# evandez/neuron-descriptions

Hardware: AMD Instinct MI355X
Metric: neuron-descriptions/sec (whole node), 4096 neurons x k=15 exemplars (higher is better)
Workload: dtype f32-equivalent: operands split into (hi,lo) f16 pairs (22 significant bits), 3 f16 MFMAs per product, f32 accumulate

## Files before the change

include/milan_hip.h:

```cpp
#ifndef MILAN_HIP_H
#define MILAN_HIP_H

#include <stddef.h>
#include <stdint.h>

#ifdef __cplusplus
extern "C" {
#endif

#if defined(__GNUC__)
#pragma GCC visibility push(default)
#endif

#define MILAN_ABI_VERSION 11

enum {
  MILAN_OK = 0,
  MILAN_ERR_ARG = -1,
  MILAN_ERR_SHAPE = -2,
  MILAN_ERR_STATE = -3,
  MILAN_ERR_WORKSPACE = -4,
  MILAN_ERR_NO_LM = -5
};

// ... 190 lines not shown
typedef struct milan_sketch_op {
  int32_t kind, src, dst, offset, extremes, reserved;
  int64_t n, position, capacity;
} milan_sketch_op;
int milan_exemplar_sketch_plan_shift(int64_t resolution, int64_t buffersize,
                                     int full_rate, int n_levels,
                                     const int64_t* capacities,
                                     const int64_t* firstfree,
                                     int (*draw_bit)(void*), void* user,
                                     milan_sketch_op* ops, int max_ops, int* n_ops,
                                     int64_t* capacities_out, int64_t* firstfree_out,
                                     int* n_levels_out);

int milan_exemplar_sketch_quantile(const float* const* levels,
                                   const int64_t* firstfree,
                                   const int64_t* capacities, int n_levels,
                                   int n_units, float* extremes, float q,
                                   float* out, void* workspace,
                                   size_t workspace_bytes, milan_stream stream);

int milan_exemplar_render(const float* hiddens, int batch, int channels, int h,
                          int w, const float* images, int img_h, int img_w,
                          const int32_t* cells, int n_cells, const float* levels,
                          const float* mul3, const float* add3, int out_size,
                          int k, uint8_t* out_images, uint8_t* out_masks,
                          uint8_t* out_masked, milan_stream stream);

int milan_conv2d_nhwc(const float* x, int n, int h, int w, int cin,
                      const float* weight_oihw, const float* bias, int cout,
                      int kh, int kw, int stride, int pad, int relu,
                      const float* residual, float* y, int precision,
                      milan_stream stream);

size_t milan_lm_train_workspace_bytes(const milan_ctx* ctx, int rows, int L);
int milan_lm_nll(milan_ctx* ctx, const float* const* params, int n_params,
                 const int64_t* inputs, const int64_t* targets, int rows, int L,
                 float* loss_sum_and_count, void* workspace,
                 size_t workspace_bytes, milan_stream stream);
int milan_lm_train_step(milan_ctx* ctx, const float* const* params,
                        float* const* grads, int n_params,
                        const int64_t* inputs, const int64_t* targets, int rows,
                        int L, float dropout, uint64_t seed,
                        float* loss_sum_and_count, void* workspace,
                        size_t workspace_bytes, milan_stream stream);

size_t milan_decoder_train_workspace_bytes(const milan_ctx* ctx, int rows,
                                           int k, int L);
int milan_decoder_nll(milan_ctx* ctx, const float* const* params, int n_params,
                      const float* features, const int64_t* targets, int rows,
                      int k, int L, float* loss_terms, void* workspace,
                      size_t workspace_bytes, milan_stream stream);
int milan_decoder_train_step(milan_ctx* ctx, const float* const* params,
                             float* const* grads, int n_params,
                             const float* features, const int64_t* targets,
                             int rows, int k, int L, float dropout,
                             uint64_t seed, float regularization_weight,
                             float* loss_terms, void* workspace,
                             size_t workspace_bytes, milan_stream stream);

size_t milan_decoder_grad_workspace_bytes(const milan_ctx* ctx, int rows, int k,
                                          int L);
int milan_decoder_forward_train(milan_ctx* ctx, const float* const* params,
                                int n_params, const float* features,
                                const int64_t* targets, int rows, int k, int L,
                                float dropout, uint64_t seed,
                                float* logprobs_out, float* attentions_out,
// ... 63 lines not shown
```

neuron-descriptions_amd/csrc/api.hip:

```cpp
#include "common.h"

#include <cstdarg>
#include <cstdio>
#include <cstring>

namespace milan {

static thread_local char g_err[1024] = "";

void set_error(const char* fmt, ...) {
  va_list ap;
  va_start(ap, fmt);
  vsnprintf(g_err, sizeof(g_err), fmt, ap);
  va_end(ap);
}

int dev_alloc(milan_ctx* c, void** p, size_t bytes) {
  if (bytes == 0) bytes = 16;
  MILAN_CHECK_HIP(hipMalloc(p, (bytes + 255) & ~size_t(255)));
  c->owned.push_back(*p);
  return 0;
}

__global__ void absmax_kernel(const float* __restrict__ w, long n,
// ... 333 lines not shown
    for (auto& g : c->graphs)
      if (g.exec) (void)hipGraphExecDestroy(g.exec);
    c->graphs.clear();
  }
  return 0;
}

int milan_graph_stats(const milan_ctx* c, long long* captures, long long* replays) {
  MILAN_REQUIRE(c, MILAN_ERR_ARG, "null ctx");
  if (captures) *captures = c->graph_captures;
  if (replays) *replays = c->graph_replays;
  return 0;
}

int milan_lm_score(milan_ctx* c, const int64_t* seqs, int rows, int L,
                   const int32_t* seq_len, float* out, void* workspace,
                   size_t workspace_bytes, milan_stream stream) {
  MILAN_REQUIRE(c && seqs && out, MILAN_ERR_ARG, "milan_lm_score: null argument");
  set_status_word(c->status);
  Arena a;
  MILAN_TRY(make_arena(workspace, workspace_bytes, &a));
  return decoder_lm_score(c, seqs, rows, L, seq_len, out, a, (hipStream_t)stream);
}

int milan_lm_logprobs(milan_ctx* c, const int64_t* seqs, int rows, int L,
                      float* out, void* workspace, size_t workspace_bytes,
                      milan_stream stream) {
  MILAN_REQUIRE(c && seqs && out, MILAN_ERR_ARG,
                "milan_lm_logprobs: null argument");
  set_status_word(c->status);
  Arena a;
  MILAN_TRY(make_arena(workspace, workspace_bytes, &a));
  return decoder_lm_logprobs(c, seqs, rows, L, out, a, (hipStream_t)stream);
}

int milan_conv2d_nhwc(const float* x, int n, int h, int w, int cin,
                      const float* weight_oihw, const float* bias, int cout,
                      int kh, int kw, int stride, int pad, int relu,
                      const float* residual, float* y, int precision,
                      milan_stream stream) {
  MILAN_REQUIRE(x && weight_oihw && y, MILAN_ERR_ARG, "conv2d: null argument");
  set_status_word(nullptr);
  const bool force_strip = precision == 3, tap_major = precision == 4;
  if (force_strip || tap_major) precision = MILAN_PRECISION_SPLIT_F16;
  MILAN_REQUIRE(!force_strip || MILAN_EXPERIMENTS, MILAN_ERR_ARG,
                "conv2d: the LDS-strip 3x3 kernel is only in an experiments build "
                "(make EXPERIMENTS=1)");
  MILAN_REQUIRE(precision == MILAN_PRECISION_F32 || cin % 32 == 0,
                MILAN_ERR_SHAPE, "conv2d: split-f16 needs cin %% 32 == 0");
  MILAN_REQUIRE(cin % 4 == 0 && n > 0 && cout > 0, MILAN_ERR_SHAPE,
                "conv2d: cin must be a multiple of 4");
  hipStream_t s = (hipStream_t)stream;
  const int K = kh * kw * cin, Kp = (K + 31) / 32 * 32;
  float *wp = nullptr, *zero = nullptr, *xs = nullptr, *wsp = nullptr, *ws3 = nullptr, *wst = nullptr;
  MILAN_CHECK_HIP(hipMalloc((void**)&wp, sizeof(float) * (size_t)cout * Kp));
  MILAN_CHECK_HIP(hipMalloc((void**)&zero, 256));
  MILAN_CHECK_HIP(hipMemsetAsync(zero, 0, 256, s));
  int r = pack_conv_plain(weight_oihw, cout, cin, kh, kw, wp, s);
  if (r == 0) {
    GemmArgs g{};
    const int ho = (h + 2 * pad - kh) / stride + 1, wo = (w + 2 * pad - kw) / stride + 1;
    g.A = x; g.W = wp; g.bias = bias; g.aux = residual; g.C = y;
    g.M = n * ho * wo; g.N = cout; g.K = K; g.Kp = Kp; g.ldc = cout; g.ldaux = cout;
    g.H = h; g.Wd = w; g.Cin = cin; g.Ho = ho; g.Wo = wo; g.KH = kh; g.KW = kw;
    g.stride = stride; g.pad = pad; g.a_pix_stride = cin;
    g.a_img_stride = (long)h * w * cin;
// ... 175 lines not shown
```

neuron-descriptions_amd/csrc/common.h:

```cpp
#pragma once
#include <hip/hip_runtime.h>
#include <stdint.h>
#include <stddef.h>
#include <string>
#include <vector>
#include <map>

#include "../../include/milan_hip.h"

#ifndef MILAN_EXPERIMENTS
#define MILAN_EXPERIMENTS 0
#endif

namespace milan {

void set_error(const char* fmt, ...);
#define MILAN_CHECK_HIP(expr)                                              \
  do {                                                                     \
    hipError_t _e = (expr);                                                \
    if (_e != hipSuccess) {                                                \
      milan::set_error("%s:%d: %s -> %s", __FILE__, __LINE__, #expr,       \
                       hipGetErrorString(_e));                             \
      return (int)_e;                                                      \
    }                                                                      \
// ... 373 lines not shown
int dev_alloc(milan_ctx* c, void** p, size_t bytes);
int make_split_weight(milan_ctx* c, const float* w, int n, int kp, float** ws,
                      float* ws_inv, hipStream_t s);
int pack_conv_plain(const float* w_oihw, int cout, int cin, int kh, int kw,
                    float* wp, hipStream_t s);
int encoder_finalize(milan_ctx* c, hipStream_t s);
int encoder_rescale(milan_ctx* c, hipStream_t s);
int make_slice_major(const float* ws, int cout, int taps, int cin, int gps, int gb, float* dst,
                     hipStream_t s);
int make_chunk_major(const float* ws, int cout, int cin, float* dst,
                     hipStream_t s);
size_t encoder_workspace(const milan_ctx* c, int n_images, int H, int W);
int encoder_run_spatial(milan_ctx* c, const void* images, int image_dtype,
                        const void* masks, int mask_dtype, int n, int H, int W,
                        float* out, milan::Arena& ws, hipStream_t s);
int encoder_run(milan_ctx* c, const void* images, int image_dtype,
                const void* masks, int mask_dtype, int n_images, int H, int W,
                float* features, Arena& ws, hipStream_t s);
int decoder_finalize(milan_ctx* c, hipStream_t s);
size_t decoder_workspace(const milan_ctx* c, int n, int k, int beam, int length);
int decoder_init_state(milan_ctx* c, const float* features, int n, int k,
                       float* h, float* cc, Arena& ws, hipStream_t s);
int decoder_step(milan_ctx* c, const float* features, int rows, int k,
                 const int64_t* tokens, const float* h, const float* cc,
                 float* h_lm, float* c_lm, float temperature,
                 float* predictions, float* attentions, float* h_out,
                 float* c_out, Arena& ws, hipStream_t s);
int decoder_decode(milan_ctx* c, const float* features, int n, int k,
                   int strategy, int length, int beam, int mi,
                   float temperature, int group_size, int64_t* tokens,
                   float* scores, float* predictions, float* attentions,
                   int64_t* beam_tokens, float* beam_scores, int32_t* out_len,
                   Arena& ws, hipStream_t s);
int decoder_lm_logprobs(milan_ctx* c, const int64_t* seqs, int rows, int L,
                        float* out, milan::Arena& ws, hipStream_t s);
int decoder_lm_score(milan_ctx* c, const int64_t* seqs, int rows, int L,
                     const int32_t* seq_len, float* out, Arena& ws,
                     hipStream_t s);
}
```

neuron-descriptions_amd/csrc/decoder.hip:

```cpp
#include "common.h"
#include <limits>
#include <optional>

namespace milan {

static constexpr float kFloatMin = -3.402823466e+38f;

static const Tensor* find(milan_ctx* c, const std::string& name) {
  auto it = c->raw.find(name);
  return it == c->raw.end() ? nullptr : &it->second;
}

__global__ void pack_rows_kernel(const float* __restrict__ src, int n, int k,
                                 int kp, float* __restrict__ dst) {
  const long total = (long)n * kp;
  for (long idx = blockIdx.x * (long)blockDim.x + threadIdx.x; idx < total;
       idx += (long)gridDim.x * blockDim.x) {
    const int r = idx / kp, col = idx - (long)r * kp;
    dst[idx] = col < k ? src[(long)r * k + col] : 0.f;
  }
}

__device__ inline int lstm_source_row(int i, int hidden) {
  if (!hidden) return i;
  const int gate = (i & 63) >> 4, u = (i >> 6) * 16 + (i & 15);
  return gate * hidden + u;
}
__global__ void add_vec_kernel(const float* a, const float* b, int n,
                               float* out, int hidden = 0) {
  const int i = blockIdx.x * blockDim.x + threadIdx.x;
  if (i < n) {
    const int r = lstm_source_row(i, hidden);
    out[i] = a[r] + (b ? b[r] : 0.f);
// ... 567 lines not shown
    sy = block_sum(sy, red);
    const float lsy = logf(sy);
    for (int i = tid; i < V; i += 256)
      pred[i] = ((pred[i] - mx) - ls) - lambda * ((y[i] - my) - lsy);
  } else {
    for (int i = tid; i < V; i += 256) pred[i] = (pred[i] - mx) - ls;
  }
  if (pred_out) {
    float* po = pred_out + (long)r * pred_stride;
    for (int i = tid; i < V; i += 256) po[i] = pred[i];
  }
  if (k <= 0) return;
  __syncthreads();
  if (last_tok && last_tok[r] == stop) {
    for (int j = tid; j < k; j += 256) {
      cand_v[(long)r * k + j] = j == 0 ? 0.f : kFloatMin;
      cand_i[(long)r * k + j] = j == 0 ? stop : (j - 1 < stop ? j - 1 : j);
    }
    return;
  }
  if (k >= 2 && k <= 256)
    block_topk_fast(pred, V, k, cand_v + (long)r * k, cand_i + (long)r * k,
                    reinterpret_cast<unsigned*>(sm + V + 8));
  else
    block_topk(pred, V, k, cand_v + (long)r * k, cand_i + (long)r * k, red, redi);
}

constexpr int kRowRegs = 24;

__device__ inline float funkey(unsigned key) {
  return __uint_as_float((key & 0x80000000u) ? (key ^ 0x80000000u) : ~key);
}

__global__ __launch_bounds__(256) void row_select_reg_kernel(
    const float* __restrict__ logits, const float* __restrict__ lm_logits,
    float lambda, int V, int k, const int64_t* __restrict__ last_tok, int stop,
    float* __restrict__ cand_v, int* __restrict__ cand_i,
    float* __restrict__ pred_out, long pred_stride, int rank_select) {
  __shared__ float red[8];
  __shared__ unsigned scratch[528];
  const int r = blockIdx.x, tid = threadIdx.x;
  const float* x = logits + (long)r * V;
  float p[kRowRegs];
  float mx = -INFINITY;
#pragma unroll
  for (int j = 0; j < kRowRegs; ++j) {
    const int i = tid + 256 * j;
    p[j] = i < V ? x[i] : -INFINITY;
    mx = fmaxf(mx, p[j]);
  }
  mx = block_max(mx, red);
  float s = 0.f;
#pragma unroll
  for (int j = 0; j < kRowRegs; ++j)
    if (tid + 256 * j < V) s += expf(p[j] - mx);
  s = block_sum(s, red);
  const float ls = logf(s);
  if (lm_logits) {
    const float* y = lm_logits + (long)r * V;
    float q[kRowRegs];
    float my = -INFINITY;
#pragma unroll
    for (int j = 0; j < kRowRegs; ++j) {
      const int i = tid + 256 * j;
      q[j] = i < V ? y[i] : -INFINITY;
      my = fmaxf(my, q[j]);
    }
// ... 5 lines not shown
    sy = block_sum(sy, red);
    const float lsy = logf(sy);
#pragma unroll
    for (int j = 0; j < kRowRegs; ++j)
      p[j] = ((p[j] - mx) - ls) - lambda * ((q[j] - my) - lsy);
  } else {
#pragma unroll
    for (int j = 0; j < kRowRegs; ++j) p[j] = (p[j] - mx) - ls;
  }
  if (pred_out) {
    float* po = pred_out + (long)r * pred_stride;
#pragma unroll
    for (int j = 0; j < kRowRegs; ++j)
      if (tid + 256 * j < V) po[tid + 256 * j] = p[j];
  }
  if (k <= 0) return;
  float* out_v = cand_v + (long)r * k;
  int* out_i = cand_i + (long)r * k;
  if (last_tok && last_tok[r] == stop) {
    for (int j = tid; j < k; j += 256) {
      out_v[j] = j == 0 ? 0.f : kFloatMin;
      out_i[j] = j == 0 ? stop : (j - 1 < stop ? j - 1 : j);
    }
    return;
  }
  unsigned key[kRowRegs];
#pragma unroll
  for (int j = 0; j < kRowRegs; ++j)
    key[j] = tid + 256 * j < V ? fkey(p[j]) : 0u;
  unsigned* cnt = scratch;
  float* cv = reinterpret_cast<float*>(scratch + 8);
  int* ci = reinterpret_cast<int*>(scratch + 8 + 256);
  if (k >= 2) {
    __shared__ unsigned gk[kGatherCap];
    __shared__ float gp[kGatherCap];
    __shared__ int gi[kGatherCap];
    __shared__ unsigned wave_t[4], gcount;
    unsigned tmax = 0u;
#pragma unroll
    for (int j = 0; j < kRowRegs; ++j) tmax = max(tmax, key[j]);
    const int m_need = (k + 3) >> 2;
    const int lane = tid & 63;
    int rank = 0;
#pragma unroll
    for (int u = 0; u < 64; ++u) {
      const unsigned m = (unsigned)__builtin_amdgcn_readlane((int)tmax, u);
      rank += (m > tmax) || (m == tmax && u < lane);
    }
    if (tid == 0) gcount = 0u;
    if (rank == m_need - 1) wave_t[tid >> 6] = rank_select ? tmax : 0u;
    __syncthreads();
    const unsigned T0 = min(min(wave_t[0], wave_t[1]), min(wave_t[2], wave_t[3]));
    if (T0 != 0u) {
#pragma unroll
      for (int j = 0; j < kRowRegs; ++j)
        if (key[j] >= T0) {
          const unsigned q = atomicAdd(&gcount, 1u);
          if (q < (unsigned)kGatherCap) { gk[q] = key[j]; gp[q] = p[j]; gi[q] = tid + 256 * j; }
        }
      __syncthreads();
      const int total = (int)gcount;
      if (total <= kGatherCap) {
        for (int c0 = tid; c0 < total; c0 += 256) {
          const unsigned mk = gk[c0];
          const int mi = gi[c0];
          int r2 = 0;
          for (int u = 0; u < total; ++u) {
            const unsigned ok = gk[u];
            r2 += (ok > mk) || (ok == mk && gi[u] < mi);
          }
          if (r2 < k) { out_v[r2] = gp[c0]; out_i[r2] = mi; }
        }
        return;
      }
    }
    __syncthreads();
  }
  unsigned kmax = 0u, kmin = 0xFFFFFFFFu;
#pragma unroll
  for (int j = 0; j < kRowRegs; ++j)
    if (tid + 256 * j < V) { kmax = max(kmax, key[j]); kmin = min(kmin, key[j]); }
  for (int o = 32; o > 0; o >>= 1) {
    kmax = max(kmax, (unsigned)__shfl_xor((int)kmax, o));
    kmin = min(kmin, (unsigned)__shfl_xor((int)kmin, o));
  }
  __syncthreads();
  if ((tid & 63) == 0) { cnt[tid >> 6] = kmax; cnt[4 + (tid >> 6)] = kmin; }
  __syncthreads();
  unsigned hi = max(max(cnt[0], cnt[1]), max(cnt[2], cnt[3]));
  unsigned lo = min(min(cnt[4], cnt[5]), min(cnt[6], cnt[7]));
  if (k == 1) {
    int best = 0x7fffffff;
#pragma unroll
    for (int j = 0; j < kRowRegs; ++j)
      if (key[j] == hi && tid + 256 * j < V) best = min(best, tid + 256 * j);
    for (int o = 32; o > 0; o >>= 1) best = min(best, __shfl_xor(best, o));
    __syncthreads();
    if ((tid & 63) == 0) cnt[tid >> 6] = (unsigned)best;
    __syncthreads();
    if (tid == 0) {
      out_i[0] = (int)min(min(cnt[0], cnt[1]), min(cnt[2], cnt[3]));
      out_v[0] = funkey(hi);
    }
    return;
  }
  for (int it = 0; it < 32 && lo < hi; ++it) {
// ... 563 lines not shown
                                      w.n, w.k, EPI_BIAS, c->zero);
      if (cell) { g.C2 = cn; g.Cs = hs2; }
      g.a_split = 1;
      g.acc_scale = w.ws_inv;
      g.Cin = ldx;
      g.A2 = hs; g.K1 = ldx; g.H2 = 1; g.W2d = 1; g.stride2 = 1;
      g.a2_pix_stride = H; g.a2_img_stride = H;
      MILAN_TRY(launch_gemm(g, s));
      if (!cell) {
        hipLaunchKernelGGL(lstm_pointwise_kernel, dim3(nblk((long)rows * H)),
                           dim3(256), 0, s, b->gates, cc, rows, H, hn, cn);
        hs2 = hs;
        MILAN_TRY(launch_f32_to_split(hn, H, hs2, H, rows, H, 1.f, s));
      }
    }
    hs = hs2;
    MILAN_TRY(launch_gemm(split_lin(c->out, b->logits, V, EPI_BIAS, nullptr, 0), s));
    MILAN_CHECK_HIP(hipGetLastError());
    return 0;
  }
  MILAN_TRY(lin(c, h, H, c->q2h, b->q, A, rows, EPI_BIAS, s));
  launch_attend(b->q, keys, c->att_w, c->att_b, rows, rpn, k, A, b->att, s);
  launch_context(b->att, features, rows, rpn, k, F, b->ctx, s);
  MILAN_TRY(lin(c, h, H, c->gate, b->x + E, ldx, rows, EPI_BIAS_SIGMUL, s, b->ctx, F));
  hipLaunchKernelGGL(embed_kernel, dim3(nblk((long)rows * E)), dim3(256), 0, s,
                     c->embedding, tok, rows, E, b->x, ldx);
  MILAN_TRY(lstm_layer(c, b->x, ldx, c->lstm_ih, h, H, c->lstm_hh, c->lstm_cat,
                       b->gates, cc, hn, cn, rows, s));
  MILAN_TRY(lin(c, hn, H, c->out, b->logits, V, rows, EPI_BIAS, s));
  MILAN_CHECK_HIP(hipGetLastError());
  return 0;
}

static size_t row_select_lds(int V) { return sizeof(float) * (V + 8 + 528); }

static int launch_row_select(const float* logits, const float* lm_logits,
                             float lambda, int rows, int V, int k,
                             const int64_t* last_tok, int stop, float* cand_v,
                             int* cand_i, float* pred_out, long pred_stride,
                             hipStream_t s) {
  if (V <= kRowRegs * 256 && k <= 256 && (k <= 1 || k <= V)) {
    static const int rank_select = [] {
      const char* e = getenv("MILAN_ROW_SELECT");
      return (e && e[0] == 't') ? 0 : 1;
    }();
    hipLaunchKernelGGL(row_select_reg_kernel, dim3(rows), dim3(256), 0, s,
                       logits, lm_logits, lambda, V, k, last_tok, stop, cand_v,
                       cand_i, pred_out, pred_stride, rank_select);
    MILAN_CHECK_HIP(hipGetLastError());
    return 0;
  }
  const size_t lds = row_select_lds(V);
  MILAN_REQUIRE(lds <= 160 * 1024, MILAN_ERR_SHAPE,
                "vocab_size %d too large for the row-select kernel", V);
  if (lds > 64 * 1024)
    MILAN_TRY(ensure_lds_attr(reinterpret_cast<const void*>(row_select_kernel), (int)lds));
  hipLaunchKernelGGL(row_select_kernel, dim3(rows), dim3(256), lds, s, logits,
                     lm_logits, lambda, V, k, last_tok, stop, cand_v, cand_i,
                     pred_out, pred_stride);
  MILAN_CHECK_HIP(hipGetLastError());
  return 0;
}

int decoder_step(milan_ctx* c, const float* features, int rows, int k,
                 const int64_t* tokens, const float* h, const float* cc,
                 float* h_lm, float* c_lm, float temperature, float* predictions,
                 float* attentions, float* h_out, float* c_out, Arena& ws,
                 hipStream_t s) {
  MILAN_TRY(check_dims(c, k));
  const bool mi = h_lm != nullptr;
  MILAN_REQUIRE((h_lm == nullptr) == (c_lm == nullptr), MILAN_ERR_ARG,
                "state must have both h_lm and c_lm or neither");
  MILAN_REQUIRE(!mi || c->d.has_lm, MILAN_ERR_NO_LM,
                "state has h_lm or c_lm, but decoder has no lm");
  DecBuf b;
  dec_plan(c, rows, k, 1, 1, mi, ws, &b);
  c->scratch = ws.off <= ws.size ? b.scratch : nullptr;
  c->scratch_floats = b.scratch_floats;
  MILAN_REQUIRE(ws.off <= ws.size, MILAN_ERR_WORKSPACE,
                "step: workspace too small (%zu needed)", ws.off);
  MILAN_TRY(project_keys(c, features, rows * k, b.keys, s));
  MILAN_TRY(step_core(c, features, b.keys, rows, 1, k, tokens, h, cc, h_out,
                      c_out, &b, s));
  const float* lm_logits = nullptr;
  if (mi) {
    LmState st{h_lm, c_lm, rows};
    MILAN_TRY(lm_step(c, tokens, rows, st, b.lm[0], b.lm_emb, b.lm_gates,
                      b.lm_logits, s));
    const size_t bytes = sizeof(float) * (size_t)rows * c->d.lm_hidden_size *
                         c->d.lm_layers;
    MILAN_CHECK_HIP(hipMemcpyAsync(h_lm, b.lm[0].h, bytes, hipMemcpyDeviceToDevice, s));
    MILAN_CHECK_HIP(hipMemcpyAsync(c_lm, b.lm[0].c, bytes, hipMemcpyDeviceToDevice, s));
    lm_logits = b.lm_logits;
  }
// ... 183 lines not shown
  const size_t state = (2 * (size_t)d.lm_layers + 1) * R * d.lm_hidden_size;
  return maps + state + 4 * R + 2048;
}

static int lm_score_dedup(milan_ctx* c, const int64_t* seqs, int rows, int L, int group,
                          const int32_t* seq_len, int len_div, float* total, DecBuf* b,
                          float* scratch, hipStream_t s) {
  const milan_dims& d = c->d;
  const int Hl = d.lm_hidden_size, El = d.lm_embedding_size, V = d.vocab_size;
  const int R = rows, G = (rows + group - 1) / group, nb = (V + 63) / 64;
  char* base = reinterpret_cast<char*>(scratch);
  size_t off = 0;
  auto take = [&](size_t bytes) { void* q = base + off; off += (bytes + 255) & ~size_t(255); return q; };
  int* rep = (int*)take(sizeof(int) * (size_t)(L + 1) * R);
  int* lrank = (int*)take(sizeof(int) * (size_t)(L + 1) * R);
  int* cnt = (int*)take(sizeof(int) * (size_t)(L + 1) * G);
  int* offs = (int*)take(sizeof(int) * (size_t)(L + 1) * G);
  LmDedup q;
  q.cls = (int*)take(sizeof(int) * (size_t)(L + 1) * R);
  q.urow = (int*)take(sizeof(int) * (size_t)(L + 1) * R);
  q.par = (int*)take(sizeof(int) * (size_t)(L + 1) * R);
  q.U = (int*)take(sizeof(int) * (size_t)(L + 1));
  q.gh = (float*)take(sizeof(float) * (size_t)d.lm_layers * R * Hl);
  q.gc = (float*)take(sizeof(float) * (size_t)d.lm_layers * R * Hl);
  q.gv = (float*)take(sizeof(float) * (size_t)R * Hl);
  q.tok_c = (int64_t*)take(sizeof(int64_t) * (size_t)R);
  q.tgt_c = (int64_t*)take(sizeof(int64_t) * (size_t)R);
  hipLaunchKernelGGL(lm_prefix_classes_kernel, dim3(G), dim3(256), 0, s, seqs, L, group, R, G,
                     rep, lrank, cnt);
  hipLaunchKernelGGL(lm_prefix_scan_kernel, dim3(L + 1), dim3(256), 0, s, cnt, G, offs, q.U);
  hipLaunchKernelGGL(lm_prefix_assign_kernel, dim3(nblk(R)), dim3(256), 0, s, rep, lrank, offs,
                     L, group, R, G, q.cls, q.urow, q.par);
  MILAN_CHECK_HIP(hipGetLastError());
  const size_t st_floats = (size_t)d.lm_layers * R * Hl;
  MILAN_TRY(launch_zero_fill(q.gh, sizeof(float) * st_floats, s));
  MILAN_TRY(launch_zero_fill(q.gc, sizeof(float) * st_floats, s));
  float* hs = b->lm_gates;
  float* emb_s = c->scratch;
  const size_t layer_sz = (size_t)R * Hl;
  int cur = 0;
  for (int t = 0; t + 1 < L; ++t) {
    const int p1 = t + 1, p2 = t + 2;
    const int* U1 = q.U + p1;
    const int* U2 = q.U + p2;
    LmState& st = b->lm[cur];
    LmState& nx = b->lm[cur ^ 1];
    hipLaunchKernelGGL(lm_gather_tok_kernel, dim3(nblk(R)), dim3(256), 0, s, seqs, (long)L, t,
                       q.urow + (size_t)p1 * R, U1, q.tok_c);
    hipLaunchKernelGGL(embed_split_kernel, dim3(nblk((long)R * (El / 8))), dim3(256), 0, s,
                       c->lm_embedding, q.tok_c, R, El, emb_s, El, U1);
    if (t > 0) {
      for (int l = 0; l < d.lm_layers; ++l) {
        hipLaunchKernelGGL(lm_gather_rows_kernel, dim3(nblk((long)R * (Hl / 4), 8192)), dim3(256),
                           0, s, (const float4*)(hs + ((size_t)cur * d.lm_layers + l) * layer_sz),
                           q.par + (size_t)p1 * R, U1, Hl / 4, (float4*)(q.gh + l * layer_sz));
        hipLaunchKernelGGL(lm_gather_rows_kernel, dim3(nblk((long)R * (Hl / 4), 8192)), dim3(256),
                           0, s, (const float4*)(st.c + (long)l * st.rows * Hl),
                           q.par + (size_t)p1 * R, U1, Hl / 4, (float4*)(q.gc + l * layer_sz));
      }
    }
    const float* in = emb_s;
    int in_dim = El;
    for (int l = 0; l < d.lm_layers; ++l) {
      float* h_next = hs + ((size_t)(cur ^ 1) * d.lm_layers + l) * layer_sz;
      float* hn = nx.h + (long)l * nx.rows * Hl;
      float* cn = nx.c + (long)l * nx.rows * Hl;
      const LinearW& w = c->lm_cat[l];
      GemmArgs g = linear_args(in, in_dim, w.ws, w.b, hn, Hl, R, w.n, w.k, EPI_LSTM, c->zero,
                               q.gc + l * layer_sz, Hl);
      g.C2 = cn; g.Cs = h_next;
      g.a_split = 1;
      g.acc_scale = w.ws_inv;
// ... 9 lines not shown
                       (const float4*)in, q.par + (size_t)p2 * R, U2, Hl / 4, (float4*)q.gv);
    hipLaunchKernelGGL(lm_gather_tok_kernel, dim3(nblk(R)), dim3(256), 0, s, seqs, (long)L, t + 1,
                       q.urow + (size_t)p2 * R, U2, q.tgt_c);
    {
      GemmArgs g = linear_args(q.gv, Hl, c->lm_out.ws, c->lm_out.b, b->lm_logits, V, R,
                               c->lm_out.n, c->lm_out.k, EPI_BIAS, c->zero);
      g.a_split = 1;
      g.acc_scale = c->lm_out.ws_inv;
      g.epilogue = EPI_LSE;
      g.ldc = 2 * nb;
      g.lse_tgt = reinterpret_cast<const long long*>(q.tgt_c);
      g.lse_tgt_stride = 1;
      g.lse_x = b->lm_logits + (size_t)R * 2 * nb;
      g.m_live = U2; g.m_live_mul = 1;
      MILAN_TRY(launch_gemm(g, s));
    }
    hipLaunchKernelGGL(lm_accumulate_lse_kernel, dim3((R + 3) / 4), dim3(256), 0, s,
                       b->lm_logits, nb, b->lm_logits + (size_t)R * 2 * nb, R, seqs, (long)L, t,
                       seq_len, len_div, d.stop_index, b->lm_alive, total,
                       q.cls + (size_t)p2 * R);
    cur ^= 1;
  }
  MILAN_CHECK_HIP(hipGetLastError());
  return 0;
}

static int lm_score_impl(milan_ctx* c, const int64_t* seqs, int rows, int L,
                         const int32_t* seq_len, int len_div, float* total,
                         DecBuf* b, hipStream_t s, int group = 1,
                         float* dedup_scratch = nullptr, size_t dedup_floats = 0) {
  const milan_dims& d = c->d;
  MILAN_REQUIRE(d.has_lm && c->lm_out.w, MILAN_ERR_NO_LM,
                "cannot use MI/rerank decoding without an LM");
  const size_t st_bytes =
      sizeof(float) * (size_t)b->lm[0].rows * d.lm_hidden_size * d.lm_layers;
  MILAN_TRY(launch_zero_fill(b->lm[0].h, st_bytes, s));
  MILAN_TRY(launch_zero_fill(b->lm[0].c, st_bytes, s));
  if (L < 2) {
    MILAN_TRY(launch_zero_fill(total, sizeof(float) * rows, s));
    return 0;
  }
  int cur = 0;
  const bool split = lm_split_ok(c, rows) && (long)rows == b->lm[0].rows;
  static const bool lse_on = !(getenv("MILAN_LM_LSE") && atoi(getenv("MILAN_LM_LSE")) == 0);
  const bool lse = lse_on && d.vocab_size % 4 == 0 && d.vocab_size >= 256;
  if (split)
    MILAN_TRY(launch_zero_fill(b->lm_gates, sizeof(float) * (size_t)rows * d.lm_hidden_size * d.lm_layers, s));
  static const bool dedup_on = !(getenv("MILAN_LM_DEDUP") && atoi(getenv("MILAN_LM_DEDUP")) == 0);
  if (dedup_on && split && lse && group > 1 && group <= 256 && rows % group == 0 && dedup_scratch &&
      d.lm_hidden_size % 4 == 0 &&
      lm_dedup_floats(d, (size_t)rows, L, rows / group) <= dedup_floats)
    return lm_score_dedup(c, seqs, rows, L, group, seq_len, len_div, total, b, dedup_scratch, s);
  for (int t = 0; t + 1 < L; ++t) {
    hipLaunchKernelGGL(gather_col_kernel, dim3(nblk(rows)), dim3(256), 0, s, seqs,
                       (long)rows, (long)L, t, b->tok);
    if (split && lse) {
      const int nb = (d.vocab_size + 63) / 64;
      MILAN_TRY(lm_step_split(c, b->tok, rows, b->lm[cur], b->lm[cur ^ 1],
                              b->lm_gates, cur, b->lm_logits, s, seqs + t + 1, (long)L));
      hipLaunchKernelGGL(lm_accumulate_lse_kernel, dim3((rows + 3) / 4), dim3(256), 0, s,
                         b->lm_logits, nb, b->lm_logits + (size_t)rows * 2 * nb, rows, seqs,
                         (long)L, t, seq_len, len_div, d.stop_index, b->lm_alive, total);
      cur ^= 1;
      continue;
    }
    if (split)
      MILAN_TRY(lm_step_split(c, b->tok, rows, b->lm[cur], b->lm[cur ^ 1],
                              b->lm_gates, cur, b->lm_logits, s));
    else
      MILAN_TRY(lm_step(c, b->tok, rows, b->lm[cur], b->lm[cur ^ 1], b->lm_emb,
                        b->lm_gates, b->lm_logits, s));
    hipLaunchKernelGGL(lm_accumulate_kernel, dim3(rows), dim3(256), 0, s,
                       b->lm_logits, d.vocab_size, seqs, (long)L, t, seq_len,
                       len_div, d.stop_index, b->lm_alive, total);
    cur ^= 1;
  }
  MILAN_CHECK_HIP(hipGetLastError());
  return 0;
}

int decoder_lm_score(milan_ctx* c, const int64_t* seqs, int rows, int L,
                     const int32_t* seq_len, float* out, Arena& ws,
                     hipStream_t s) {
  MILAN_REQUIRE(c->finalized, MILAN_ERR_STATE, "weights not finalized");
  MILAN_REQUIRE(c->d.has_lm && c->lm_out.w, MILAN_ERR_NO_LM,
// ... 194 lines not shown
```

neuron-descriptions_amd/milan_amd/hip.py:

```python
import ctypes
import os
import pathlib
import weakref
from typing import Dict, Optional, Sequence

import torch

LIB_PATH = pathlib.Path(os.environ.get('MILAN_LIB') or
                       pathlib.Path(__file__).resolve().parent / 'lib' / 'libmilan_hip.so')
EXP_LIB_PATH = pathlib.Path(__file__).resolve().parent / 'lib' / 'libmilan_hip_exp.so'

GREEDY, FORCED, BEAM, RERANK = 0, 1, 2, 3
PRECISION_F32, PRECISION_SPLIT_F16, PRECISION_F16 = 0, 1, 2
PRECISIONS = {'f32': PRECISION_F32, 'split_f16': PRECISION_SPLIT_F16, 'f16': PRECISION_F16}
FUSE_CHAIN, FUSE_CHAIN_WIDE, FUSE_STEM, FUSE_CONV3, FUSE_SKIP_EMPTY, FUSE_BNECK, FUSE_SPARSE_TAIL = 1, 2, 4, 8, 16, 32, 64
SKETCH_COMPACT, SKETCH_INSERT, SKETCH_MOVE, SKETCH_HALVE = 0, 1, 2, 3
STATUS_SATURATED, STATUS_NONFINITE_INPUT = 1, 2
KERNEL_FAMILIES = ('other', 'pp32_256', 'pp32_128', 'split_other', 'f32', 'chain',
                   'chain_wide', 'stem', 'conv3', 'f16', 'pp32t_256', 'bneck')


class SketchOp(ctypes.Structure):
    _fields_ = [('kind', ctypes.c_int32), ('src', ctypes.c_int32),
                ('dst', ctypes.c_int32), ('offset', ctypes.c_int32),
# ... 127 lines not shown
    'milan_lm_train_workspace_bytes': (_SZ, [_P, _I, _I]),
    'milan_lm_nll': (_I, [_P, _P, _I, _P, _P, _I, _I, _P, _P, _SZ, _P]),
    'milan_lm_train_step':
        (_I, [_P, _P, _P, _I, _P, _P, _I, _I, _F, ctypes.c_uint64, _P, _P,
              _SZ, _P]),
    'milan_decoder_train_workspace_bytes': (_SZ, [_P, _I, _I, _I]),
    'milan_decoder_nll':
        (_I, [_P, _P, _I, _P, _P, _I, _I, _I, _P, _P, _SZ, _P]),
    'milan_decoder_train_step':
        (_I, [_P, _P, _P, _I, _P, _P, _I, _I, _I, _F, ctypes.c_uint64, _F, _P,
              _P, _SZ, _P]),
    'milan_decoder_grad_workspace_bytes': (_SZ, [_P, _I, _I, _I]),
    'milan_decoder_forward_train':
        (_I, [_P, _P, _I, _P, _P, _I, _I, _I, _F, ctypes.c_uint64, _P, _P, _P,
              _SZ, _P]),
    'milan_decoder_backward':
        (_I, [_P, _P, _P, _I, _P, _P, _I, _I, _I, _F, ctypes.c_uint64, _P, _P,
              _P, _P, _SZ, _P]),
    'milan_clip_create': (_I, [ctypes.POINTER(_P), _I,
                               ctypes.POINTER(ClipDims)]),
    'milan_clip_destroy': (None, [_P]),
    'milan_clip_set_weight':
        (_I, [_P, ctypes.c_char_p, _P,
              ctypes.POINTER(ctypes.c_int64), _I]),
    'milan_clip_finalize_weights': (_I, [_P, _P]),
    'milan_clip_image_workspace_bytes': (_SZ, [_P, _I, _I]),
    'milan_clip_encode_images':
        (_I, [_P, _P, _I, _I, _P, ctypes.c_uint64, _I,
              ctypes.POINTER(_F), _P, _P, _SZ, _P]),
    'milan_clip_text_workspace_bytes': (_SZ, [_P, _I, _I]),
    'milan_clip_encode_texts': (_I, [_P, _P, _I, _I, _P, _P, _SZ, _P]),
    'milan_clip_rerank_scores':
        (_I, [_P, _P, _P, _P, _I, _I, _I, _I, _I, _F, _P, _P]),
    'milan_conv2d_nhwc':
        (_I, [_P, _I, _I, _I, _I, _P, _P, _I, _I, _I, _I, _I, _I, _P, _P, _I,
              _P]),
}

_lib = None


def load_library(path: Optional[os.PathLike] = None) -> ctypes.CDLL:
    global _lib
    if _lib is not None and path is None:
        return _lib
    p = pathlib.Path(path) if path is not None else LIB_PATH
    if not p.exists():
        raise HipUnavailableError(
            f'{p} not found: build it with `python -c "import __graft_entry__ '
            'as g; g.build()"` (or `make -C neuron-descriptions_amd/csrc`). '
            'There is no CPU fallback for the MILAN hot path.')
    try:
        lib = ctypes.CDLL(str(p))
    except OSError as error:
        raise HipUnavailableError(f'cannot load {p}: {error}') from error
    for name, (restype, argtypes) in SIGNATURES.items():
        fn = getattr(lib, name)
        fn.restype = restype
        fn.argtypes = argtypes
    if lib.milan_abi_version() != ABI_VERSION:
        raise HipUnavailableError(
            f'{p} has C-ABI version {lib.milan_abi_version()}, this binding '
            f'needs {ABI_VERSION} (struct milan_dims differs): rebuild it')
    if path is None:
        _lib = lib
    return lib
# ... 955 lines not shown
    table = (ctypes.c_double * (len(KERNEL_FAMILIES) * 4))()
    _check(load_library().milan_profile_read_kernels(table))
    keys = ('ms', 'flops', 'launches', 'bytes')
    return {name: dict(zip(keys, table[i * 4:i * 4 + 4]))
            for i, name in enumerate(KERNEL_FAMILIES)}


def conv2d_nhwc(x: torch.Tensor,
                weight: torch.Tensor,
                bias: Optional[torch.Tensor] = None,
                stride: int = 1,
                padding: int = 0,
                relu: bool = False,
                residual: Optional[torch.Tensor] = None,
                precision: str = 'f32',
                lib: Optional[ctypes.CDLL] = None) -> torch.Tensor:
    lib = lib if lib is not None else load_library()
    device = require_device(x.device)
    n, h, w, cin = x.shape
    cout, cin_w, kh, kw = weight.shape
    assert cin_w == cin
    ho = (h + 2 * padding - kh) // stride + 1
    wo = (w + 2 * padding - kw) // stride + 1
    y = torch.empty(n, ho, wo, cout, device=device)
    x, weight = x.contiguous(), weight.contiguous()
    with torch.cuda.device(device):
        _check(
            lib.milan_conv2d_nhwc(x.data_ptr(), n, h, w, cin,
                                  weight.data_ptr(), _ptr(bias), cout, kh, kw,
                                  stride, padding, int(relu), _ptr(residual),
                                  y.data_ptr(), _CONV_PRECISIONS[precision],
                                  _stream(device)))
    return y


def make_dims(state_dict: Dict[str, torch.Tensor],
              n_vocab_tokens: int,
              blocks: Sequence[int] = (3, 4, 23, 3)) -> Dims:
    d = Dims()
    sd = state_dict
    pre = 'encoder.encoder.model.'
    width = kind = None
    if pre + 'features.0.weight' in sd:
        kind, width = TRUNK_ALEXNET, sd[pre + 'features.0.weight'].shape[0]
    elif pre + 'conv1.weight' in sd:
        width = sd[pre + 'conv1.weight'].shape[0]
        kind = (TRUNK_BOTTLENECK if pre + 'layer1.0.conv3.weight' in sd else
                TRUNK_BASIC)
    if 'lstm.weight_hh' in sd:
        hidden = sd['lstm.weight_hh'].shape[1]
        emb = sd['embedding.weight'].shape[1]
        feat = sd['lstm.weight_ih'].shape[1] - emb
        att = sd['attend.query_to_hidden.weight'].shape[0]
        vocab = sd['output.1.weight'].shape[0]
    else:
        hidden, emb, att, vocab = 4, 4, 4, n_vocab_tokens + 4
        feat = _FEATURE_MULT[kind] * width if kind is not None else 4
    if width is None:
        if feat % 4:
            raise ValueError(f'feature size {feat} must be a multiple of 4')
        kind, width = TRUNK_NONE, 0
    d.trunk_kind = kind
    if vocab != n_vocab_tokens + 4:
        raise ValueError(
            f'output layer has {vocab} classes but the indexer has '
            f'{n_vocab_tokens} tokens + 4 specials')
# ... 18 lines not shown
```

Baseline: 1340.

## Add ballot-based row-select threshold, packed-key parallel rank, and trim LM state zero-fills

Adds a templated ballot path for the decoder's top-k row selection and makes it the default. It finds the per-wave threshold by bitwise binary search with ballots instead of 64 readlanes per lane. Candidates are packed into 64-bit key|index words and ranked in parallel across split partitions. Separately, LM-score zero-fills are moved past the dedup early return, and the dedup path zeroes only the rows it uses, cutting redundant memset traffic. The change also exposes a standalone row_select API for testing modes, and adds a launch_bounds occupancy hint that may raise register pressure.

```diff
diff --git a/include/milan_hip.h b/include/milan_hip.h
--- a/include/milan_hip.h
+++ b/include/milan_hip.h
@@ -246,6 +246,11 @@
                       const float* residual, float* y, int precision,
                       milan_stream stream);
 
+int milan_row_select(const float* logits, const float* lm_logits, float lambda,
+                     int rows, int V, int k, const int64_t* last_tok, int stop,
+                     float* cand_v, int32_t* cand_i, float* pred_out, int mode,
+                     milan_stream stream);
+
 size_t milan_lm_train_workspace_bytes(const milan_ctx* ctx, int rows, int L);
 int milan_lm_nll(milan_ctx* ctx, const float* const* params, int n_params,
                  const int64_t* inputs, const int64_t* targets, int rows, int L,
diff --git a/neuron-descriptions_amd/csrc/api.hip b/neuron-descriptions_amd/csrc/api.hip
--- a/neuron-descriptions_amd/csrc/api.hip
+++ b/neuron-descriptions_amd/csrc/api.hip
@@ -389,6 +389,16 @@
   Arena a;
   MILAN_TRY(make_arena(workspace, workspace_bytes, &a));
   return decoder_lm_logprobs(c, seqs, rows, L, out, a, (hipStream_t)stream);
+}
+
+int milan_row_select(const float* logits, const float* lm_logits, float lambda,
+                     int rows, int V, int k, const int64_t* last_tok, int stop,
+                     float* cand_v, int32_t* cand_i, float* pred_out, int mode,
+                     milan_stream stream) {
+  MILAN_REQUIRE(logits, MILAN_ERR_ARG, "milan_row_select: null argument");
+  set_status_word(nullptr);
+  return decoder_row_select(logits, lm_logits, lambda, rows, V, k, last_tok, stop,
+                            cand_v, cand_i, pred_out, mode, (hipStream_t)stream);
 }
 
 int milan_conv2d_nhwc(const float* x, int n, int h, int w, int cin,
diff --git a/neuron-descriptions_amd/csrc/common.h b/neuron-descriptions_amd/csrc/common.h
--- a/neuron-descriptions_amd/csrc/common.h
+++ b/neuron-descriptions_amd/csrc/common.h
@@ -429,6 +429,10 @@
                    float* scores, float* predictions, float* attentions,
                    int64_t* beam_tokens, float* beam_scores, int32_t* out_len,
                    Arena& ws, hipStream_t s);
+int decoder_row_select(const float* logits, const float* lm_logits, float lambda,
+                       int rows, int V, int k, const int64_t* last_tok, int stop,
+                       float* cand_v, int* cand_i, float* pred_out, int mode,
+                       hipStream_t s);
 int decoder_lm_logprobs(milan_ctx* c, const int64_t* seqs, int rows, int L,
                         float* out, milan::Arena& ws, hipStream_t s);
 int decoder_lm_score(milan_ctx* c, const int64_t* seqs, int rows, int L,
diff --git a/neuron-descriptions_amd/csrc/decoder.hip b/neuron-descriptions_amd/csrc/decoder.hip
--- a/neuron-descriptions_amd/csrc/decoder.hip
+++ b/neuron-descriptions_amd/csrc/decoder.hip
@@ -1,4 +1,5 @@
 #include "common.h"
+#include <algorithm>
 #include <limits>
 #include <optional>
 
@@ -632,7 +633,8 @@
   return __uint_as_float((key & 0x80000000u) ? (key ^ 0x80000000u) : ~key);
 }
 
-__global__ __launch_bounds__(256) void row_select_reg_kernel(
+template <bool kBallot>
+__global__ __launch_bounds__(256, 4) void row_select_reg_kernel(
     const float* __restrict__ logits, const float* __restrict__ lm_logits,
     float lambda, int V, int k, const int64_t* __restrict__ last_tok, int stop,
     float* __restrict__ cand_v, int* __restrict__ cand_i,
@@ -704,46 +706,98 @@
   float* cv = reinterpret_cast<float*>(scratch + 8);
   int* ci = reinterpret_cast<int*>(scratch + 8 + 256);
   if (k >= 2) {
-    __shared__ unsigned gk[kGatherCap];
-    __shared__ float gp[kGatherCap];
-    __shared__ int gi[kGatherCap];
     __shared__ unsigned wave_t[4], gcount;
     unsigned tmax = 0u;
 #pragma unroll
     for (int j = 0; j < kRowRegs; ++j) tmax = max(tmax, key[j]);
     const int m_need = (k + 3) >> 2;
-    const int lane = tid & 63;
-    int rank = 0;
-#pragma unroll
-    for (int u = 0; u < 64; ++u) {
-      const unsigned m = (unsigned)__builtin_amdgcn_readlane((int)tmax, u);
-      rank += (m > tmax) || (m == tmax && u < lane);
-    }
-    if (tid == 0) gcount = 0u;
-    if (rank == m_need - 1) wave_t[tid >> 6] = rank_select ? tmax : 0u;
+    if constexpr (kBallot) {
+      unsigned t = 0u;
+      for (int bit = 31; bit >= 0; --bit) {
+        const unsigned cand = t | (1u << bit);
+        if (__popcll(__ballot(tmax >= cand)) >= m_need) t = cand;
+      }
+      if (tid == 0) gcount = 0u;
+      if ((tid & 63) == 0) wave_t[tid >> 6] = rank_select ? t : 0u;
+    } else {
+      const int lane = tid & 63;
+      int rank = 0;
+#pragma unroll
+      for (int u = 0; u < 64; ++u) {
+        const unsigned m = (unsigned)__builtin_amdgcn_readlane((int)tmax, u);
+        rank += (m > tmax) || (m == tmax && u < lane);
+      }
+      if (tid == 0) gcount = 0u;
+      if (rank == m_need - 1) wave_t[tid >> 6] = rank_select ? tmax : 0u;
+    }
     __syncthreads();
     const unsigned T0 = min(min(wave_t[0], wave_t[1]), min(wave_t[2], wave_t[3]));
-    if (T0 != 0u) {
-#pragma unroll
-      for (int j = 0; j < kRowRegs; ++j)
-        if (key[j] >= T0) {
-          const unsigned q = atomicAdd(&gcount, 1u);
-          if (q < (unsigned)kGatherCap) { gk[q] = key[j]; gp[q] = p[j]; gi[q] = tid + 256 * j; }
+    if constexpr (kBallot) {
+      if (T0 != 0u) {
+        __shared__ unsigned long long gw[kGatherCap];
+#pragma unroll
+        for (int j = 0; j < kRowRegs; ++j)
+          if (key[j] >= T0) {
+            const unsigned q = atomicAdd(&gcount, 1u);
+            if (q < (unsigned)kGatherCap)
+              gw[q] = ((unsigned long long)key[j] << 32) | (unsigned)~(tid + 256 * j);
+          }
+        __syncthreads();
+        const int total = (int)gcount;
+        if (total <= kGatherCap) {
+          const int lgP = total <= 64 ? 6 : total <= 128 ? 7 : 8;
+          const int P = 1 << lgP, lgsplit = 8 - lgP;
+          const int len = (total + (1 << lgsplit) - 1) >> lgsplit;
+          const int u0 = __builtin_amdgcn_readfirstlane((tid >> lgP) * len);
+          const int u1 = min(total, u0 + len);
+          unsigned* part = scratch;
+          for (int c0 = tid & (P - 1), pass = 0; c0 < total; c0 += P, ++pass) {
+            const unsigned long long mine = gw[c0];
+            unsigned r2 = 0;
+#pragma unroll 4
+            for (int u = u0; u < u1; ++u) r2 += gw[u] > mine;
+            part[pass * 256 + tid] = r2;
+          }
+          __syncthreads();
+          if (tid < P)
+            for (int c0 = tid, pass = 0; c0 < total; c0 += P, ++pass) {
+              unsigned r2 = 0;
+              for (int q = 0; q < (1 << lgsplit); ++q) r2 += part[pass * 256 + (q << lgP) + tid];
+              if (r2 < (unsigned)k) {
+                const unsigned long long w = gw[c0];
+                out_v[r2] = funkey((unsigned)(w >> 32));
+                out_i[r2] = (int)~(unsigned)w;
+              }
+            }
+          return;
         }
-      __syncthreads();
-      const int total = (int)gcount;
-      if (total <= kGatherCap) {
-        for (int c0 = tid; c0 < total; c0 += 256) {
-          const unsigned mk = gk[c0];
-          const int mi = gi[c0];
-          int r2 = 0;
-          for (int u = 0; u < total; ++u) {
-            const unsigned ok = gk[u];
-            r2 += (ok > mk) || (ok == mk && gi[u] < mi);
+      }
+    } else {
+      __shared__ unsigned gk[kGatherCap];
+      __shared__ float gp[kGatherCap];
+      __shared__ int gi[kGatherCap];
+      if (T0 != 0u) {
+#pragma unroll
+        for (int j = 0; j < kRowRegs; ++j)
+          if (key[j] >= T0) {
+            const unsigned q = atomicAdd(&gcount, 1u);
+            if (q < (unsigned)kGatherCap) { gk[q] = key[j]; gp[q] = p[j]; gi[q] = tid + 256 * j; }
           }
-          if (r2 < k) { out_v[r2] = gp[c0]; out_i[r2] = mi; }
+        __syncthreads();
+        const int total = (int)gcount;
+        if (total <= kGatherCap) {
+          for (int c0 = tid; c0 < total; c0 += 256) {
+            const unsigned mk = gk[c0];
+            const int mi = gi[c0];
+            int r2 = 0;
+            for (int u = 0; u < total; ++u) {
+              const unsigned ok = gk[u];
+              r2 += (ok > mk) || (ok == mk && gi[u] < mi);
+            }
+            if (r2 < k) { out_v[r2] = gp[c0]; out_i[r2] = mi; }
+          }
+          return;
         }
-        return;
       }
     }
     __syncthreads();
@@ -1373,21 +1427,29 @@
   return 0;
 }
 
+enum { ROW_SELECT_THRESHOLD = 0, ROW_SELECT_READLANE = 1, ROW_SELECT_BALLOT = 2 };
+
 static size_t row_select_lds(int V) { return sizeof(float) * (V + 8 + 528); }
 
 static int launch_row_select(const float* logits, const float* lm_logits,
                              float lambda, int rows, int V, int k,
                              const int64_t* last_tok, int stop, float* cand_v,
                              int* cand_i, float* pred_out, long pred_stride,
-                             hipStream_t s) {
+                             hipStream_t s, int mode = -1) {
   if (V <= kRowRegs * 256 && k <= 256 && (k <= 1 || k <= V)) {
-    static const int rank_select = [] {
+    if (mode < 0) {
       const char* e = getenv("MILAN_ROW_SELECT");
-      return (e && e[0] == 't') ? 0 : 1;
-    }();
-    hipLaunchKernelGGL(row_select_reg_kernel, dim3(rows), dim3(256), 0, s,
-                       logits, lm_logits, lambda, V, k, last_tok, stop, cand_v,
-                       cand_i, pred_out, pred_stride, rank_select);
+      mode = (e && e[0] == 't') ? ROW_SELECT_THRESHOLD
+                                : (e && e[0] == 'r') ? ROW_SELECT_READLANE : ROW_SELECT_BALLOT;
+    }
+    if (mode == ROW_SELECT_BALLOT)
+      hipLaunchKernelGGL(row_select_reg_kernel<true>, dim3(rows), dim3(256), 0, s,
+                         logits, lm_logits, lambda, V, k, last_tok, stop, cand_v,
+                         cand_i, pred_out, pred_stride, 1);
+    else
+      hipLaunchKernelGGL(row_select_reg_kernel<false>, dim3(rows), dim3(256), 0, s,
+                         logits, lm_logits, lambda, V, k, last_tok, stop, cand_v,
+                         cand_i, pred_out, pred_stride, mode == ROW_SELECT_READLANE);
     MILAN_CHECK_HIP(hipGetLastError());
     return 0;
   }
@@ -1401,6 +1463,20 @@
                      pred_out, pred_stride);
   MILAN_CHECK_HIP(hipGetLastError());
   return 0;
+}
+
+int decoder_row_select(const float* logits, const float* lm_logits, float lambda,
+                       int rows, int V, int k, const int64_t* last_tok, int stop,
+                       float* cand_v, int* cand_i, float* pred_out, int mode,
+                       hipStream_t s) {
+  MILAN_REQUIRE(rows > 0 && V > 0 && k >= 0 && k <= V, MILAN_ERR_SHAPE,
+                "row_select: rows=%d V=%d k=%d", rows, V, k);
+  MILAN_REQUIRE(mode >= -1 && mode <= ROW_SELECT_BALLOT, MILAN_ERR_ARG,
+                "row_select: unknown mode %d", mode);
+  MILAN_REQUIRE(k == 0 || (cand_v && cand_i), MILAN_ERR_ARG,
+                "row_select: k > 0 needs cand_v and cand_i");
+  return launch_row_select(logits, lm_logits, lambda, rows, V, k, last_tok, stop,
+                           cand_v, cand_i, pred_out, V, s, mode);
 }
 
 int decoder_step(milan_ctx* c, const float* features, int rows, int k,
@@ -1650,12 +1726,14 @@
   hipLaunchKernelGGL(lm_prefix_assign_kernel, dim3(nblk(R)), dim3(256), 0, s, rep, lrank, offs,
                      L, group, R, G, q.cls, q.urow, q.par);
   MILAN_CHECK_HIP(hipGetLastError());
-  const size_t st_floats = (size_t)d.lm_layers * R * Hl;
-  MILAN_TRY(launch_zero_fill(q.gh, sizeof(float) * st_floats, s));
-  MILAN_TRY(launch_zero_fill(q.gc, sizeof(float) * st_floats, s));
   float* hs = b->lm_gates;
   float* emb_s = c->scratch;
   const size_t layer_sz = (size_t)R * Hl;
+  const size_t zero_rows = std::min<size_t>((size_t)R, ((size_t)G + 255) / 256 * 256);
+  for (int l = 0; l < d.lm_layers; ++l) {
+    MILAN_TRY(launch_zero_fill(q.gh + l * layer_sz, sizeof(float) * zero_rows * Hl, s));
+    MILAN_TRY(launch_zero_fill(q.gc + l * layer_sz, sizeof(float) * zero_rows * Hl, s));
+  }
   int cur = 0;
   for (int t = 0; t + 1 < L; ++t) {
     const int p1 = t + 1, p2 = t + 2;
@@ -1731,10 +1809,6 @@
   const milan_dims& d = c->d;
   MILAN_REQUIRE(d.has_lm && c->lm_out.w, MILAN_ERR_NO_LM,
                 "cannot use MI/rerank decoding without an LM");
-  const size_t st_bytes =
-      sizeof(float) * (size_t)b->lm[0].rows * d.lm_hidden_size * d.lm_layers;
-  MILAN_TRY(launch_zero_fill(b->lm[0].h, st_bytes, s));
-  MILAN_TRY(launch_zero_fill(b->lm[0].c, st_bytes, s));
   if (L < 2) {
     MILAN_TRY(launch_zero_fill(total, sizeof(float) * rows, s));
     return 0;
@@ -1743,13 +1817,17 @@
   const bool split = lm_split_ok(c, rows) && (long)rows == b->lm[0].rows;
   static const bool lse_on = !(getenv("MILAN_LM_LSE") && atoi(getenv("MILAN_LM_LSE")) == 0);
   const bool lse = lse_on && d.vocab_size % 4 == 0 && d.vocab_size >= 256;
-  if (split)
-    MILAN_TRY(launch_zero_fill(b->lm_gates, sizeof(float) * (size_t)rows * d.lm_hidden_size * d.lm_layers, s));
   static const bool dedup_on = !(getenv("MILAN_LM_DEDUP") && atoi(getenv("MILAN_LM_DEDUP")) == 0);
   if (dedup_on && split && lse && group > 1 && group <= 256 && rows % group == 0 && dedup_scratch &&
       d.lm_hidden_size % 4 == 0 &&
       lm_dedup_floats(d, (size_t)rows, L, rows / group) <= dedup_floats)
     return lm_score_dedup(c, seqs, rows, L, group, seq_len, len_div, total, b, dedup_scratch, s);
+  const size_t st_bytes =
+      sizeof(float) * (size_t)b->lm[0].rows * d.lm_hidden_size * d.lm_layers;
+  MILAN_TRY(launch_zero_fill(b->lm[0].h, st_bytes, s));
+  MILAN_TRY(launch_zero_fill(b->lm[0].c, st_bytes, s));
+  if (split)
+    MILAN_TRY(launch_zero_fill(b->lm_gates, sizeof(float) * (size_t)rows * d.lm_hidden_size * d.lm_layers, s));
   for (int t = 0; t + 1 < L; ++t) {
     hipLaunchKernelGGL(gather_col_kernel, dim3(nblk(rows)), dim3(256), 0, s, seqs,
                        (long)rows, (long)L, t, b->tok);
diff --git a/neuron-descriptions_amd/milan_amd/hip.py b/neuron-descriptions_amd/milan_amd/hip.py
--- a/neuron-descriptions_amd/milan_amd/hip.py
+++ b/neuron-descriptions_amd/milan_amd/hip.py
@@ -183,6 +183,8 @@
     'milan_clip_encode_texts': (_I, [_P, _P, _I, _I, _P, _P, _SZ, _P]),
     'milan_clip_rerank_scores':
         (_I, [_P, _P, _P, _P, _I, _I, _I, _I, _I, _F, _P, _P]),
+    'milan_row_select':
+        (_I, [_P, _P, _F, _I, _I, _I, _P, _I, _P, _P, _P, _I, _P]),
     'milan_conv2d_nhwc':
         (_I, [_P, _I, _I, _I, _I, _P, _P, _I, _I, _I, _I, _I, _I, _P, _P, _I,
               _P]),
@@ -1204,6 +1206,37 @@
                                   y.data_ptr(), _CONV_PRECISIONS[precision],
                                   _stream(device)))
     return y
+
+
+ROW_SELECT_MODES = {'env': -1, 'threshold': 0, 'readlane': 1, 'ballot': 2}
+
+
+def row_select(logits: torch.Tensor,
+               k: int,
+               lm_logits: Optional[torch.Tensor] = None,
+               temperature: float = 0.0,
+               last_tok: Optional[torch.Tensor] = None,
+               stop: int = 0,
+               want_pred: bool = False,
+               mode: str = 'env'):
+    device = require_device(logits.device)
+    rows, v = logits.shape
+    logits = logits.contiguous()
+    if lm_logits is not None:
+        lm_logits = lm_logits.contiguous()
+    if last_tok is not None:
+        last_tok = last_tok.to(torch.long).contiguous()
+    cand_v = torch.empty(rows, k, device=device)
+    cand_i = torch.empty(rows, k, dtype=torch.int32, device=device)
+    pred = torch.empty(rows, v, device=device) if want_pred else None
+    with torch.cuda.device(device):
+        _check(
+            load_library().milan_row_select(
+                logits.data_ptr(), _ptr(lm_logits), float(temperature), rows, v,
+                k, _ptr(last_tok), stop, _ptr(cand_v) if k else None,
+                _ptr(cand_i) if k else None, _ptr(pred),
+                ROW_SELECT_MODES[mode], _stream(device)))
+    return cand_v, cand_i, pred
 
 
 def make_dims(state_dict: Dict[str, torch.Tensor],
```

Result: no change. 1347 (median of 6 runs) (+0.5%).
